# 3169651074/real-time-gpu-ray-tracer

Measured on AMD Instinct MI355X. Metric: Mrays/sec + ms/frame, 1920×1080 1spp primary+shadow, 1/2/4/8 MI355X, higher is better.
Workload: dtype f32; 1 GPU; C2: demo + 68x1024 tris (69,632; bunny stand-in), 1080p 1spp primary+shadow; width=1920, height=1080, spp=1, depth=2, triangles=69633, instances=73, blas_node_pairs=69159, parallelism=single-gpu, overlap_lanes=4, lane_streams=the scene's own (overlap -1: lanes and staging picked by the library), hw_queues=4, tile=32, threshold=auto (64 at depth x spp <= 2, else 40), kernel=FAST persistent, bvh=sah, frames=animated (Main.cu updateInstance), per-frame TLAS rebuild + upload, pipelined

## Files before the change

### real-time-gpu-ray-tracer_amd/csrc/layout.hpp

```cpp
#pragma once
#include <stdint.h>

#include "../../include/rt.h"

namespace rtamd {

constexpr uint32_t REF_LEAF = 1u << 31;
constexpr uint32_t REF_BLAS = 1u << 30;
constexpr uint32_t REF_INDEX_MASK = (1u << 30) - 1u;
constexpr uint32_t REF_START_MASK = (1u << 26) - 1u;
constexpr uint32_t REF_EMPTY = 0xFFFFFFFFu;
constexpr uint32_t MAX_LEAF_SLOTS = 1u << 26;

__host__ __device__ inline uint32_t make_interior_ref(uint32_t pair, bool blas) {
    return (blas ? REF_BLAS : 0u) | (pair & REF_INDEX_MASK);
}
__host__ __device__ inline uint32_t make_leaf_ref(uint32_t start, uint32_t count, uint32_t ptype, bool blas) {
    return REF_LEAF | (blas ? REF_BLAS : 0u) | ((ptype & 3u) << 28) | (((count - 1u) & 3u) << 26) |
           (start & REF_START_MASK);
}
__host__ __device__ inline uint32_t ref_leaf_start(uint32_t r) { return r & REF_START_MASK; }
__host__ __device__ inline uint32_t ref_leaf_count(uint32_t r) { return ((r >> 26) & 3u) + 1u; }
__host__ __device__ inline uint32_t ref_leaf_type(uint32_t r) { return (r >> 28) & 3u; }

// ... 146 lines not shown

constexpr uint32_t FASTDIV_BITS = 27;
struct FastDiv {
    uint32_t d, m, s;
    __host__ __device__ uint32_t div(uint32_t n) const { return (uint32_t)(((uint64_t)n * m) >> s); }
};
inline FastDiv make_fastdiv(uint32_t d) {
    uint32_t l = 0;
    while (l < 31 && (1u << l) < d) l++;
    const uint32_t s = FASTDIV_BITS + l;
    return FastDiv{d, (uint32_t)(((1ull << s) + d - 1) / d), s};
}

struct OutputGPU {
    uint8_t *rgba;
    float *rgb;
    uint32_t units;
    uint32_t units_x;
    uint32_t tile_w, tile_h, tile_rank, tile_count, tiles_x;
    FastDiv div_units_x, div_upt, div_upr, div_tiles_x;
    uint32_t queue_parts;
    uint32_t grab;
    uint32_t supertile;
    unsigned long long *timeline;
    uint32_t *costmap;
    const uint32_t *order;
    uint32_t *unit_cost;
    uint32_t leaf_early;
};
struct RayQueryGPU {
    const float *rays;
    const float *tmax;
    uint32_t n;
    rt_hit *hits;
    float *t;
    uint8_t *occluded;
    uint32_t *head;
};
constexpr uint32_t QUERY_PARTS = 8;
constexpr uint32_t QUEUE_STRIDE = 32;
constexpr uint32_t QUEUE_MAX_PARTS = 8;
constexpr uint32_t QUEUE_WORDS = 2 * QUEUE_MAX_PARTS * QUEUE_STRIDE;
constexpr uint32_t SCHED_CLASSES = 16;

__host__ __device__ inline uint32_t cost_class(uint32_t c) {
    const uint64_t x = (uint64_t)c + 64u;
    const int k = (63 - __builtin_clzll(x * x)) - 12;
    return (SCHED_CLASSES - 1) - (uint32_t)(k < 0 ? 0 : (k > (int)SCHED_CLASSES - 1 ? (int)SCHED_CLASSES - 1 : k));
}
__host__ __device__ inline uint32_t split_log2(uint32_t cls, uint32_t k_half, uint32_t k_quarter) {
    const uint32_t k = (SCHED_CLASSES - 1) - cls;
    return k >= k_quarter ? 2u : (k >= k_half ? 1u : 0u);
}
constexpr uint32_t TIMELINE_WORDS = 20;

enum CounterSlot : uint32_t {
    CNT_RAYS = 0, CNT_PIXELS, CNT_PAIRS, CNT_TRI, CNT_SPHQUAD, CNT_QUAD, CNT_INST, CNT_HITS, CNT_OVERFLOW, CNT_NUM
};

}
```

### real-time-gpu-ray-tracer_amd/csrc/shade.hpp

```cpp

struct Surface { f3 p, n; uint32_t material; uint32_t orig; uint32_t member; };

template <bool LDSS = false, int RAW = 2>
__device__ __forceinline__ Surface finalize(const SceneGPU &sc, const f3 &wo, const f3 &wd, const Hit &h) {
#if !RT_EXACT
    const InstCold IC = LDSS ? lds_or_global(sc.lds_icold, sc.inst_cold, h.inst) : sc.inst_cold[h.inst];
#else
    const InstCold &IC = sc.inst_cold[h.inst];
#endif
    f3 lo, ld;
#if !RT_EXACT
    if (LDSS) {
        const InstRec I = load_inst<true>(sc, h.inst);
        const float inv[12] = {I.i0.x, I.i0.y, I.i0.z, I.i0.w, I.i1.x, I.i1.y, I.i1.z, I.i1.w,
                               I.i2.x, I.i2.y, I.i2.z, I.i2.w};
        lo = xf_point(inv, wo); ld = xf_vector(inv, wd);
    } else
#endif
    {
        const InstHot &I = sc.inst_hot[h.inst];
        lo = xf_point(I.inv, wo); ld = xf_vector(I.inv, wd);
    }
    const f3 p = add(lo, scl(ld, h.t));
    f3 n;
    Surface s;
    if (h.ptype == RT_PRIM_TRIANGLE) {
        f3 n0, n1, n2;
        if (RAW == 1 || (RAW == 2 && sc.raw_tris)) {
            const TriHot &H = sc.tri_hot[h.slot];
            s.orig = __float_as_uint(H.pad0);
            s.member = __float_as_uint(H.pad1);
            const rt_triangle &R = sc.raw_tris[s.orig];
            if (R.has_normals) {
                n0 = mk(R.normal[0].x, R.normal[0].y, R.normal[0].z);
                n1 = mk(R.normal[1].x, R.normal[1].y, R.normal[1].z);
                n2 = mk(R.normal[2].x, R.normal[2].y, R.normal[2].z);
            } else {
                n0 = tri_face_normal(ld3(H.e1), ld3(H.e2)); n1 = n0; n2 = n0;
            }
            s.material = R.material_type == RT_MAT_ROUGH ? R.material_index
                                                         : ((sc.rough_count + R.material_index) | MAT_METAL_BIT);
        } else {
            const TriCold &T = sc.tri_cold[h.slot];
            n0 = ld3(T.n0); n1 = ld3(T.n1); n2 = ld3(T.n2);
            s.material = T.material; s.orig = T.orig_index; s.member = T.pad;
        }
        const f3 nn = unit(add(add(scl(n0, (1.0f - h.u) - h.v), scl(n1, h.u)), scl(n2, h.v)));
        n = dot(ld, nn) < 0.0f ? nn : neg(nn);
    } else if (h.ptype == RT_PRIM_SPHERE) {
#if !RT_EXACT
        const SphereHot S = LDSS ? lds_or_global(sc.lds_sph_hot, sc.sph_hot, h.slot) : sc.sph_hot[h.slot];
        const PrimCold C = LDSS ? lds_or_global(sc.lds_sph_cold, sc.sph_cold, h.slot) : sc.sph_cold[h.slot];
#else
        const SphereHot &S = sc.sph_hot[h.slot];
        const PrimCold &C = sc.sph_cold[h.slot];
#endif
        const f3 outward = unit(sub(p, ld3(S.center)));
        n = dot(ld, outward) < 0.0f ? outward : neg(outward);
        s.material = C.material; s.orig = C.orig_index; s.member = 0u;
    } else {
#if !RT_EXACT
        const float4 qn4 = LDSS && sc.lds_q_hot != LDS_NONE ? lds_scene[sc.lds_q_hot + h.slot * LDS_QPRIM_F4]
                                                              : reinterpret_cast<const float4 *>(sc.quad_hot + h.slot)[0];
        const PrimCold C = LDSS ? lds_or_global(sc.lds_q_cold, sc.quad_cold, h.slot) : sc.quad_cold[h.slot];
        const f3 qn = mk(qn4.x, qn4.y, qn4.z);
#else
        const QuadHot &Q = sc.quad_hot[h.slot];
        const PrimCold &C = sc.quad_cold[h.slot];
        const f3 qn = ld3(Q.n);
#endif
        n = dot(ld, qn) < 0.0f ? qn : neg(qn);
        s.material = C.material; s.orig = C.orig_index; s.member = 0u;
    }
    s.p = xf_point(IC.fwd, p);
    s.n = unit(xf_vector(IC.nrm, n));
    return s;
}

template <bool COUNT>
__device__ f3 ray_color(const SceneGPU &sc, const CameraGPU &cam, f3 o, f3 d, Rng &rng, Trav &T, SEnt *spill,
                        LaneCount &cnt, uint32_t &rays) {
    f3 result = mk(1.0f, 1.0f, 1.0f);
    for (uint32_t depth = 0; depth < cam.depth; depth++) {
        Hit h;
        rays++;
        if (trace<COUNT, XD_ALL>(sc, o, d, h, T, spill, cnt)) {
            if (COUNT) cnt.hits++;
            const Surface s = finalize(sc, o, d, h);
            const float4 m = reinterpret_cast<const float4 *>(sc.materials)[s.material & ~MAT_METAL_BIT];
            const f3 albedo = mk(m.x, m.y, m.z);
            f3 out;
            if (!(s.material & MAT_METAL_BIT)) {
                out = add(s.n, random_space_vector(rng));
                if (f_eq(dot(out, out), FZERO * FZERO)) out = s.n;
            } else {
                out = unit(sub(d, scl(s.n, 2.0f * dot(d, s.n))));
                if (m.w > 0.0f) out = add(out, scl(random_space_vector(rng), m.w));
                if (!(dot(out, s.n) > 0.0f)) return result;
            }
            o = s.p; d = out;
            result = mul(result, albedo);
        } else {
            result = mul(result, ld3(cam.background));
            break;
        }
    }
    return result;
}

__device__ __forceinline__ uint32_t wave_sum(uint32_t v) {
#pragma unroll
    for (int off = 32; off > 0; off >>= 1) v += __shfl_xor(v, off, 64);
    return v;
}

template <bool COUNT>
__device__ __forceinline__ void flush_counts(unsigned long long *counters, const LaneCount &cnt, int lane) {
    if (COUNT) {
        const uint32_t a = wave_sum(cnt.pairs), b = wave_sum(cnt.tri), c = wave_sum(cnt.sq), d = wave_sum(cnt.inst),
                       e = wave_sum(cnt.overflow), f = wave_sum(cnt.quad), g = wave_sum(cnt.hits);
        if (lane == 0) {
            atomicAdd(&counters[CNT_PAIRS], (unsigned long long)a);
            atomicAdd(&counters[CNT_TRI], (unsigned long long)b);
            atomicAdd(&counters[CNT_SPHQUAD], (unsigned long long)c);
            atomicAdd(&counters[CNT_INST], (unsigned long long)d);
            atomicAdd(&counters[CNT_OVERFLOW], (unsigned long long)e);
            atomicAdd(&counters[CNT_QUAD], (unsigned long long)f);
            atomicAdd(&counters[CNT_HITS], (unsigned long long)g);
        }
// ... 76 lines not shown
```

### real-time-gpu-ray-tracer_amd/csrc/trace_kernel.hip

```cpp
#include <hip/hip_runtime.h>
#include <stdint.h>

#include <atomic>

#include "launch.hpp"
#include "layout.hpp"
#include "../../include/rt.h"

#ifndef RT_EXACT
#error "compile with -DRT_EXACT=0 or 1"
#endif

#ifndef RT_FAST_IEEE
#define RT_FAST_IEEE 1
#endif
#if RT_EXACT
#define RT_SUFFIX(n) n##_exact
#elif RT_FAST_IEEE
#define RT_SUFFIX(n) n##_fast
#else
#define RT_SUFFIX(n) n##_fastmath
#endif

namespace rtamd {
// ... 200 lines not shown
                    const uint32_t m = k - sc * st * h;
                    const uint32_t u = (r0 + sr * st + m / w) * W + sc * st + m % w;
                    pool_next = u * 64u;
                    pool_end = pool_next + 64u;
                }
            }
            const uint32_t take = min(n_need, pool_end - pool_next);
            const uint32_t rank = __popcll(need & ((1ull << lane) - 1ull));
            DIAG_T(t_lanes);
            if (!has && rank < take) {
                uint32_t px, py, oi;
                item = pool_next + rank;
                if (map_item(out, cam, item, px, py, oi)) {
                    has = true;
                    const uint32_t pixel = cam.pitch * py + px;
                    rng.init((uint64_t)pixel ^ cam.frame_seed, pixel);
                    acc = mk(0.0f, 0.0f, 0.0f);
                    thr = mk(1.0f, 1.0f, 1.0f);
                    sample = 0; depth = 0;
                    px_steps = 0;
                    f3 o, d;
                    camera_ray(cam, px, py, 0, rng, o, d);
                    trav_init<XBOX(WIDE)>(T, root, o, d);
                    pixels++;
                }
            }
            DIAG_ADD(pc.claim, t_lanes);
            pool_next += take;
            need = __ballot(!has);
        }
        DIAG_ADD(pc.refill, t_refill);
        if (!__any(has)) {
            if (exhausted) break;
            continue;
        }
        for (;;) {
            const uint64_t tr = __ballot(T.tracing);
            if (tr == 0) break;
            const uint64_t want = __ballot(!T.tracing && (has || !exhausted));
            if ((uint32_t)__popcll(want) >= threshold) break;
            spec_round<COUNT, WIDE>(T, sc, spill, cnt, pc, px_steps, COUNT || track, out.leaf_early);
            n_rounds++;
        }
        n_shades++;
        DIAG_T(t_shade);
        bool fin = false;
        if (RT_DIAG) pc.lanes_shade += (unsigned long long)__popcll(__ballot(has && !T.tracing));
        if (has && !T.tracing) {
            rays++;
            bool path_done;
            f3 no = T.wr.o, nd = T.wr.d;
            if (T.found) {
                if (COUNT) cnt.hits++;
                const Surface s = finalize<WIDE != 0, RAW>(sc, T.wr.o, T.wr.d, T.hit);
                DIAG_WAIT_VM();
                DIAG_T(t_hit);
                const uint32_t mi = s.material & ~MAT_METAL_BIT;
                const float4 m = mat_lds ? lds_mat[mi] : reinterpret_cast<const float4 *>(sc.materials)[mi];
                bool absorbed = false;
                if (!(s.material & MAT_METAL_BIT)) {
                    if (depth + 1 < cam.depth || sample + 1 < S2) {
                        nd = add(s.n, random_space_vector(rng));
                        if (f_eq(dot(nd, nd), FZERO * FZERO)) nd = s.n;
                    }
                } else {
                    nd = unit(sub(T.wr.d, scl(s.n, 2.0f * dot(T.wr.d, s.n))));
                    if (m.w > 0.0f) nd = add(nd, scl(random_space_vector(rng), m.w));
                    absorbed = !(dot(nd, s.n) > 0.0f);
                }
                DIAG_ADD(pc.hit, t_hit);
                if (absorbed) {
                    path_done = true;
                } else {
                    thr = mul(thr, mk(m.x, m.y, m.z));
                    no = s.p;
                    depth++;
                    path_done = depth >= cam.depth;
                }
            } else {
                thr = mul(thr, ld3(cam.background));
                path_done = true;
            }
            if (path_done) {
                acc = add(acc, thr);
                sample++;
                uint32_t px, py, oi;
                map_item(out, cam, item, px, py, oi);
                if (sample < S2) {
                    thr = mk(1.0f, 1.0f, 1.0f);
                    depth = 0;
                    camera_ray(cam, px, py, sample, rng, no, nd);
                } else {
                    write_pixel(out, oi, scl(acc, cam.recip_sqrt * cam.recip_sqrt));
                    if (COUNT && out.costmap) out.costmap[oi] = px_steps;
                    has = false;
                    fin = true;
                }
            }
            if (has) trav_init<XBOX(WIDE)>(T, root, no, nd);
        }
        if (track && fin) {
            const uint32_t u = item >> 6;
            if (u != pend_unit) {
                if (pend_cost) unit_cost_flush(out.unit_cost, pend_unit, pend_cost);
                pend_unit = u;
                pend_cost = 0;
            }
            pend_cost = pend_cost + px_steps + 1u;
        }
        DIAG_ADD(pc.shade, t_shade);
    }

    if (track && pend_cost) unit_cost_flush(out.unit_cost, pend_unit, pend_cost);
    const uint32_t wr = wave_sum(rays);
    const uint32_t wp = wave_sum(pixels);
    flush_counts<COUNT>(counters, cnt, lane);
    if (lane == 0) {
        atomicAdd(&counters[CNT_RAYS], (unsigned long long)wr);
        atomicAdd(&counters[CNT_PIXELS], (unsigned long long)wp);
        if (out.timeline) {
            const uint32_t wv = (uint32_t)((const unsigned long long *)T.stk.lds - &lds_stack[0][0]) >> 6;
            unsigned long long *w = out.timeline + (unsigned long long)TIMELINE_WORDS * (blockIdx.x * (BLOCK / 64) + wv);
            w[0] = t_start;
            w[1] = __builtin_amdgcn_s_memrealtime();
            w[2] = ((unsigned long long)hw_id() << 32) | xcc;
            w[3] = wp;
            w[4] = t_exhaust;
            w[5] = n_rounds;
            w[6] = n_shades;
            w[7] = n_grabs;
            w[8] = pc.refill;
            w[9] = pc.interior;
            w[10] = pc.leaf;
            w[11] = pc.shade;
            w[12] = pc.iters;
            w[13] = pc.refill_iters;
            w[14] = pc.claim;
            w[15] = pc.hit;
            w[16] = pc.lanes_interior;
            w[17] = pc.lanes_leaf_tlas;
            w[18] = pc.lanes_leaf_blas;
            w[19] = pc.lanes_shade;
        }
    }
}

template <bool COUNT, int WPE, int WIDE = 0, int RAW = 2>
__global__ __launch_bounds__(BLOCK) __attribute__((amdgpu_waves_per_eu(WPE > 0 ? WPE : 1)))
void render_persistent_kernel(SceneGPU sc, CameraGPU cam, OutputGPU out, uint32_t *queue, uint32_t threshold,
                              unsigned long long *counters) {
    render_persistent_body<COUNT, WIDE, RAW>(sc, cam, out, queue, threshold, counters);
}

__global__ __launch_bounds__(BLOCK) void trace_rays_kernel(SceneGPU sc, const float *rays, uint32_t n, rt_hit *hits) {
    __shared__ unsigned long long lds_stack[LDS_DEPTH][BLOCK];
    const uint32_t i = blockIdx.x * BLOCK + threadIdx.x;
    if (i >= n) return;
    Trav T;
    T.stk.lds = (LdsU2 *)&lds_stack[0][threadIdx.x];
    alignas(16) SEnt spill[SPILL_DEPTH];
    LaneCount cnt = {};
    const f3 o = mk(rays[6 * i], rays[6 * i + 1], rays[6 * i + 2]);
    const f3 d = mk(rays[6 * i + 3], rays[6 * i + 4], rays[6 * i + 5]);
    Hit h;
    rt_hit r;
    if (trace<false, XD_ALL>(sc, o, d, h, T, spill, cnt)) {
        const Surface s = finalize(sc, o, d, h);
        r.t = h.t; r.instance = s.member ? s.member - 1u : (sc.inst_by_slot ? sc.tlas_slots[h.inst] : h.inst);
        r.primitive_type = h.ptype; r.primitive_index = s.orig;
        r.point.x = s.p.x; r.point.y = s.p.y; r.point.z = s.p.z;
        r.normal.x = s.n.x; r.normal.y = s.n.y; r.normal.z = s.n.z;
        const bool metal = (s.material & MAT_METAL_BIT) != 0;
        r.material_type = metal ? RT_MAT_METAL : RT_MAT_ROUGH;
        r.material_index = (s.material & ~MAT_METAL_BIT) - (metal ? sc.rough_count : 0u);
    } else {
        r.t = __builtin_huge_valf(); r.instance = 0xFFFFFFFFu; r.primitive_type = 0; r.primitive_index = 0;
        r.point.x = r.point.y = r.point.z = 0.0f; r.normal.x = r.normal.y = r.normal.z = 0.0f;
        r.material_type = 0; r.material_index = 0;
    }
    hits[i] = r;
}


__global__ __launch_bounds__(BLOCK) void box_test_kernel(const float *boxes, const float *rays, const float *tmaxs, uint32_t n,
                                                         uint32_t mode, uint8_t *hit, float *te) {
    const uint32_t i = blockIdx.x * BLOCK + threadIdx.x;
    if (i >= n) return;
    float b[6];
    for (int c = 0; c < 6; c++) b[c] = boxes[6 * (size_t)i + c];
    RayP r;
    r.o = mk(rays[6 * (size_t)i], rays[6 * (size_t)i + 1], rays[6 * (size_t)i + 2]);
    r.d = mk(rays[6 * (size_t)i + 3], rays[6 * (size_t)i + 4], rays[6 * (size_t)i + 5]);
    const float tmax = tmaxs[i];
    float e = 0.0f;
    bool h = false;
#if RT_EXACT
// ... 128 lines not shown
```

### real-time-gpu-ray-tracer_amd/csrc/traverse.hpp

```cpp

struct Hit {
    float t;
    uint32_t inst;
    uint32_t ptype;
    uint32_t slot;
    float u, v;
};

struct Trav {
    RayP wr, lr;
    float tmax;
    uint32_t cur;
    float curT;
    uint32_t pleaf;
    uint32_t cur_inst;
    Hit hit;
    bool found;
    bool tracing;
    Stack stk;
};

__device__ __forceinline__ bool pop_keep(const Trav &T, float tn, uint32_t ref) {
#if !RT_EXACT
    return cons_lo(tn, (ref & REF_BLAS) ? T.lr.pad : T.wr.pad) < T.tmax;
// ... 69 lines not shown
        float e0 = 0.0f, e1 = 0.0f;
        bool h0, h1;
        const uint4 D = pair_test<COUNT, XB>(T, sc, cur, cnt, h0, h1, e0, e1);
        if (h0 && h1) {
            const bool right_near = e0 > e1;
            stack_push(T.stk, spill, right_near ? D.x : D.y, right_near ? e0 : e1, cnt);
            T.cur = right_near ? D.y : D.x;
            return;
        }
        if (h0) { T.cur = D.x; return; }
        if (h1) { T.cur = D.y; return; }
    } else if (!(cur & REF_BLAS)) {
        const uint32_t start = ref_leaf_start(cur), count = ref_leaf_count(cur);
        if (count > 1) stack_push(T.stk, spill, make_leaf_ref(start + 1, count - 1, 0, false), -__builtin_huge_valf(), cnt);
        T.cur_inst = sc.inst_by_slot ? start : sc.tlas_slots[start];
        const InstHot &I = sc.inst_hot[T.cur_inst];
        if (COUNT) cnt.inst++;
        float te;
        if (enter_instance<XB>(T, I.inv, I.root_box, te)) { T.cur = I.root_ref; return; }
    } else {
        const uint32_t start = ref_leaf_start(cur), count = ref_leaf_count(cur), type = ref_leaf_type(cur);
        for (uint32_t k = 0; k < count; k++) {
            const uint32_t slot = start + k;
            float t = 0.0f, u = 0.0f, v = 0.0f;
            bool h;
            if (type == RT_PRIM_TRIANGLE) {
                if (COUNT) cnt.tri++;
                h = tri_test(sc.tri_hot[slot], T.lr, TMIN, T.tmax, t, u, v);
            } else if (type == RT_PRIM_SPHERE) {
                if (COUNT) cnt.sq++;
                h = sphere_test(sc.sph_hot[slot], T.lr, TMIN, T.tmax, t);
            } else {
                if (COUNT) { cnt.sq++; cnt.quad++; }
                h = quad_test(sc.quad_hot[slot], T.lr, TMIN, T.tmax, t, u, v);
            }
            if (h) accept(T, t, type, slot, u, v);
        }
    }
    while (!T.stk.empty()) {
        const SEnt e = stack_pop(T.stk, spill);
        if (pop_keep(T, __uint_as_float(e.tn), e.ref)) { T.cur = e.ref; return; }
    }
    T.tracing = false;
}

__device__ __forceinline__ void pop_next(Trav &T, const SEnt *spill) {
    while (!T.stk.empty()) {
        const SEnt e = stack_pop(T.stk, spill);
        const float tn = __uint_as_float(e.tn);
        if (pop_keep(T, tn, e.ref)) { T.cur = e.ref; T.curT = tn; return; }
    }
    T.cur = REF_NONE;
}

#if !RT_EXACT
__shared__ float4 lds_scene[LDS_SCENE_F4];

struct InstRec { float4 i0, i1, i2, box01, box2ref; };
template <bool LDSS>
__device__ __forceinline__ InstRec load_inst(const SceneGPU &sc, uint32_t i) {
    InstRec r;
    if (LDSS && sc.lds_insts) {
        const float4 *p = lds_scene + sc.lds_quads * LDS_QUAD_F4 + i * LDS_INST_F4;
        r.i0 = p[0]; r.i1 = p[1]; r.i2 = p[2]; r.box01 = p[3]; r.box2ref = p[4];
    } else {
        const float4 *p = reinterpret_cast<const float4 *>(sc.inst_hot + i);
        r.i0 = p[0]; r.i1 = p[1]; r.i2 = p[2]; r.box01 = p[3]; r.box2ref = p[4];
    }
    return r;
}
__device__ __forceinline__ void lds_scene_fill(const SceneGPU &sc) {
    const uint32_t nq = sc.lds_quads * LDS_QUAD_F4, ni = sc.lds_insts * LDS_INST_F4;
    const float4 *q = reinterpret_cast<const float4 *>(sc.tlas_quads);
    for (uint32_t i = threadIdx.x; i < nq; i += BLOCK) {
        const uint32_t k = i / LDS_QUAD_F4, j = i - k * LDS_QUAD_F4;
        lds_scene[i] = q[k * 8 + j];
    }
    const float4 *h = reinterpret_cast<const float4 *>(sc.inst_hot);
    for (uint32_t i = threadIdx.x; i < ni; i += BLOCK) lds_scene[nq + i] = h[i];
    const auto copy = [](uint32_t at, const void *src, uint32_t n4) {
        if (at == LDS_NONE) return;
        const float4 *p = reinterpret_cast<const float4 *>(src);
        for (uint32_t i = threadIdx.x; i < n4; i += BLOCK) lds_scene[at + i] = p[i];
    };
    copy(sc.lds_icold, sc.inst_cold, sc.instance_count * LDS_ICOLD_F4);
    copy(sc.lds_sph_hot, sc.sph_hot, sc.lds_sph_cold - sc.lds_sph_hot);
    copy(sc.lds_sph_cold, sc.sph_cold, sc.lds_sph_cold - sc.lds_sph_hot);
    copy(sc.lds_q_hot, sc.quad_hot, (sc.lds_q_cold - sc.lds_q_hot));
    copy(sc.lds_q_cold, sc.quad_cold, (sc.lds_q_cold - sc.lds_q_hot) / LDS_QPRIM_F4);
    const float4 *bq = reinterpret_cast<const float4 *>(sc.blas_quads + sc.lds_bq0);
    for (uint32_t i = threadIdx.x; i < sc.lds_bqn * LDS_QUAD_F4; i += BLOCK) {
        const uint32_t k = i / LDS_QUAD_F4, j = i - k * LDS_QUAD_F4;
        lds_scene[sc.lds_bq_at + i] = bq[k * 8 + j];
    }
}
template <typename R>
__device__ __forceinline__ R lds_or_global(uint32_t at, const R *g, uint32_t k) {
    constexpr uint32_t N4 = sizeof(R) / 16;
    R r;
    float4 *d = reinterpret_cast<float4 *>(&r);
    if (at != LDS_NONE) {
#pragma unroll
        for (uint32_t j = 0; j < N4; j++) d[j] = lds_scene[at + k * N4 + j];
    } else {
        const float4 *p = reinterpret_cast<const float4 *>(g + k);
#pragma unroll
// ... 36 lines not shown
    if (!PAIR) {
        float t0 = h[0] ? t[0] : inf, t1 = h[1] ? t[1] : inf, t2 = h[2] ? t[2] : inf, t3 = h[3] ? t[3] : inf;
        uint32_t r0 = R.x, r1 = R.y, r2 = R.z, r3 = R.w;
        const uint32_t nh = (uint32_t)h[0] + (uint32_t)h[1] + (uint32_t)h[2] + (uint32_t)h[3];
        if (nh == 0) { pop_next(T, spill); return; }
        cswap(t0, r0, t1, r1); cswap(t2, r2, t3, r3); cswap(t0, r0, t2, r2); cswap(t1, r1, t3, r3); cswap(t1, r1, t2, r2);
        if (nh > 1) {
            if (T.stk.sp > LDS_DEPTH - 3) stack_page_out(T.stk, spill, cnt);
            SEnt a, b, c;
            a.ref = nh == 4 ? r3 : (nh == 3 ? r2 : r1);
            a.tn = __float_as_uint(nh == 4 ? t3 : (nh == 3 ? t2 : t1));
            b.ref = nh == 4 ? r2 : r1;
            b.tn = __float_as_uint(nh == 4 ? t2 : t1);
            c.ref = r1;
            c.tn = __float_as_uint(t1);
            stack_push3(T.stk, a, b, c, nh - 1u);
        }
        T.cur = r0;
        T.curT = t0;
        return;
    }
    const uint32_t na = (uint32_t)h[0] + (uint32_t)h[1], nb = (uint32_t)h[2] + (uint32_t)h[3];
    if (na + nb == 0) { pop_next(T, spill); return; }
    const float u0 = h[0] ? t[0] : inf, u1 = h[1] ? t[1] : inf, u2 = h[2] ? t[2] : inf, u3 = h[3] ? t[3] : inf;
    const bool sa = u0 > u1, sb = u2 > u3;
    const float a0t = sa ? u1 : u0, a1t = sa ? u0 : u1, b0t = sb ? u3 : u2, b1t = sb ? u2 : u3;
    const uint32_t a0r = sa ? R.y : R.x, a1r = sa ? R.x : R.y, b0r = sb ? R.w : R.z, b1r = sb ? R.z : R.w;
    const bool sr = na == 0 || (nb != 0 && pa > pb);
    const float n0t = sr ? b0t : a0t, n1t = sr ? b1t : a1t, f0t = sr ? a0t : b0t, f1t = sr ? a1t : b1t;
    const uint32_t n0r = sr ? b0r : a0r, n1r = sr ? b1r : a1r, f0r = sr ? a0r : b0r, f1r = sr ? a1r : b1r;
    const uint32_t nn = sr ? nb : na, nf = sr ? na : nb;
    const uint32_t npush = nn - 1u + nf;
    if (npush > 0) {
        if (T.stk.sp > LDS_DEPTH - 3) stack_page_out(T.stk, spill, cnt);
        SEnt a, b, c;
        a.ref = nf == 2 ? f1r : (nf == 1 ? f0r : n1r);
        a.tn = __float_as_uint(nf == 2 ? f1t : (nf == 1 ? f0t : n1t));
        b.ref = nf == 2 ? f0r : n1r;
        b.tn = __float_as_uint(nf == 2 ? f0t : n1t);
        c.ref = n1r;
        c.tn = __float_as_uint(n1t);
        stack_push3(T.stk, a, b, c, npush);
    }
    T.cur = n0r;
    T.curT = n0t;
}
#endif

template <bool COUNT, int WIDE = 0>
__device__ __forceinline__ void spec_interior_step(Trav &T, const SceneGPU &sc, SEnt *spill, LaneCount &cnt) {
    const uint32_t cur = T.cur;
#if !RT_EXACT
    if (WIDE) {
        if (!(cur & REF_LEAF)) wide_interior_step<COUNT, (WIDE >= 2), XBOX(WIDE)>(T, sc, spill, cnt);
        else { T.pleaf = cur; pop_next(T, spill); }
        return;
    }
#endif
    if (!(cur & REF_LEAF)) {
        float e0 = 0.0f, e1 = 0.0f;
        bool h0, h1;
        const uint4 D = pair_test<COUNT, XBOX(WIDE)>(T, sc, cur, cnt, h0, h1, e0, e1);
        if (h0 && h1) {
            const bool right_near = e0 > e1;
            stack_push(T.stk, spill, right_near ? D.x : D.y, right_near ? e0 : e1, cnt);
            T.cur = right_near ? D.y : D.x;
            T.curT = right_near ? e1 : e0;
            return;
        }
        if (h0 || h1) {
            T.cur = h0 ? D.x : D.y;
            T.curT = h0 ? e0 : e1;
            return;
        }
        pop_next(T, spill);
    } else {
        T.pleaf = cur;
        pop_next(T, spill);
    }
}

#if RT_EXACT
#define WIDE_LDS_REC(at, arr, k) (arr)[k]
#else
#define WIDE_LDS_REC(at, arr, k) (WIDE ? lds_or_global((at), (arr), (k)) : (arr)[k])
#endif
template <bool COUNT, int WIDE = 0>
__device__ __forceinline__ uint32_t spec_leaf_phase(Trav &T, const SceneGPU &sc, SEnt *spill, LaneCount &cnt) {
    uint32_t leaf = T.pleaf;
    bool chained = false;
    T.pleaf = REF_NONE;
    if (!(leaf & REF_BLAS)) {
        const uint32_t start = ref_leaf_start(leaf), count = ref_leaf_count(leaf);
        if (T.cur != REF_NONE) stack_push(T.stk, spill, T.cur, T.curT, cnt);
        if (count > 1) stack_push(T.stk, spill, make_leaf_ref(start + 1, count - 1, 0, false), -__builtin_huge_valf(), cnt);
        T.cur_inst = sc.inst_by_slot ? start : sc.tlas_slots[start];
        if (COUNT) cnt.inst++;
        float te = 0.0f;
#if !RT_EXACT
        if (WIDE) {
            const InstRec I = load_inst<true>(sc, T.cur_inst);
            asm volatile("" ::"v"(I.i2.x), "v"(I.i2.y), "v"(I.i2.z), "v"(I.i2.w), "v"(I.box2ref.w));
            const float inv[12] = {I.i0.x, I.i0.y, I.i0.z, I.i0.w, I.i1.x, I.i1.y, I.i1.z, I.i1.w,
                                   I.i2.x, I.i2.y, I.i2.z, I.i2.w};
            const float box[6] = {I.box01.x, I.box01.y, I.box01.z, I.box01.w, I.box2ref.x, I.box2ref.y};
            if (enter_instance<XBOX(WIDE)>(T, inv, box, te)) {
                T.cur = __float_as_uint(I.box2ref.w);
                T.curT = te;
                if (RT_CHAIN_ROOT_LEAF && (T.cur & REF_LEAF)) { leaf = T.cur; chained = true; }
            } else {
                pop_next(T, spill);
            }
        } else
#endif
        {
            const InstHot &I = sc.inst_hot[T.cur_inst];
            if (enter_instance<XBOX(WIDE)>(T, I.inv, I.root_box, te)) { T.cur = WIDE ? I.root_ref_wide : I.root_ref; T.curT = te; }
            else pop_next(T, spill);
        }
    }
    if (leaf & REF_BLAS) {
        const uint32_t start = ref_leaf_start(leaf), count = ref_leaf_count(leaf), type = ref_leaf_type(leaf);
        if (type == RT_PRIM_TRIANGLE) {
            for (uint32_t k0 = 0; k0 < count; k0 += TRI_AHEAD) {
                TriHot H[TRI_AHEAD];
#pragma unroll
                for (uint32_t k = 0; k < TRI_AHEAD; k++) {
                    const float *src = sc.tri_hot[start + min(k0 + k, count - 1u)].v0;
                    const float3 a = *reinterpret_cast<const float3 *>(src);
                    const float3 b = *reinterpret_cast<const float3 *>(src + 4);
                    const float3 c = *reinterpret_cast<const float3 *>(src + 8);
                    H[k].v0[0] = a.x; H[k].v0[1] = a.y; H[k].v0[2] = a.z;
                    H[k].e1[0] = b.x; H[k].e1[1] = b.y; H[k].e1[2] = b.z;
                    H[k].e2[0] = c.x; H[k].e2[1] = c.y; H[k].e2[2] = c.z;
                }
#pragma unroll
                for (uint32_t k = 0; k < TRI_AHEAD; k++) {
                    if (k0 + k >= count) break;
                    float t = 0.0f, u = 0.0f, v = 0.0f;
                    if (COUNT) cnt.tri++;
                    if (tri_test(H[k], T.lr, TMIN, T.tmax, t, u, v)) accept(T, t, type, start + k0 + k, u, v);
                }
            }
        } else {
            for (uint32_t k = 0; k < count; k++) {
                const uint32_t slot = start + k;
                float t = 0.0f, u = 0.0f, v = 0.0f;
                bool h;
                if (type == RT_PRIM_SPHERE) {
                    if (COUNT) cnt.sq++;
                    h = sphere_test(WIDE_LDS_REC(sc.lds_sph_hot, sc.sph_hot, slot), T.lr, TMIN, T.tmax, t);
                } else {
                    if (COUNT) { cnt.sq++; cnt.quad++; }
                    h = quad_test(WIDE_LDS_REC(sc.lds_q_hot, sc.quad_hot, slot), T.lr, TMIN, T.tmax, t, u, v);
                }
                if (h) accept(T, t, type, slot, u, v);
            }
        }
        if (chained) pop_next(T, spill);
        else if (T.cur != REF_NONE && !pop_keep(T, T.curT, T.cur)) pop_next(T, spill);
    }
    if (T.cur == REF_NONE) T.tracing = false;
    return chained ? 1u : 0u;
}

#ifndef RT_DIAG
#define RT_DIAG 0
#endif
struct PhaseCycles {
    unsigned long long refill, interior, leaf, shade, iters, refill_iters, claim, hit;
    unsigned long long lanes_interior, lanes_leaf_tlas, lanes_leaf_blas, lanes_shade;
};
__device__ __forceinline__ unsigned long long stamp() {
    unsigned long long t;
    asm volatile("s_memtime %0\n\ts_waitcnt lgkmcnt(0)" : "=s"(t)::"memory");
    return t;
}
#if RT_DIAG
#define DIAG_WAIT_VM() asm volatile("s_waitcnt vmcnt(0)" ::: "memory")
#define DIAG_T(var) const unsigned long long var = stamp()
#define DIAG_ADD(acc, t0) (acc) += stamp() - (t0)
#else
#define DIAG_WAIT_VM() (void)0
#define DIAG_T(var) (void)0
#define DIAG_ADD(acc, t0) (void)0
#endif

template <bool COUNT, int WIDE = 0>
__device__ __forceinline__ void spec_round(Trav &T, const SceneGPU &sc, SEnt *spill, LaneCount &cnt,
                                           PhaseCycles &pc, uint32_t &steps, bool track, uint32_t leaf_early) {
    DIAG_T(t0);
    for (;;) {
        if (T.tracing && T.pleaf == REF_NONE && T.cur == REF_NONE) T.tracing = false;
        const uint64_t looking = __ballot(T.tracing && T.pleaf == REF_NONE);
        if (!looking) break;
        if (leaf_early && (uint32_t)__popcll(looking) <= leaf_early && __any(T.tracing && T.pleaf != REF_NONE)) break;
        const bool active = T.tracing && T.cur != REF_NONE && (!(T.cur & REF_LEAF) || T.pleaf == REF_NONE);
        if (RT_DIAG) pc.lanes_interior += (unsigned long long)__popcll(__ballot(active));
        if (active) {
            spec_interior_step<COUNT, WIDE>(T, sc, spill, cnt);
            if (track) steps++;
        }
        if (RT_DIAG) pc.iters++;
    }
    DIAG_ADD(pc.interior, t0);
    if (RT_DIAG) {
        pc.lanes_leaf_tlas += (unsigned long long)__popcll(__ballot(T.tracing && T.pleaf != REF_NONE && !(T.pleaf & REF_BLAS)));
        pc.lanes_leaf_blas += (unsigned long long)__popcll(__ballot(T.tracing && T.pleaf != REF_NONE && (T.pleaf & REF_BLAS)));
    }
    DIAG_T(t1);
    if (T.tracing && T.pleaf != REF_NONE) {
        const uint32_t chained = spec_leaf_phase<COUNT, WIDE>(T, sc, spill, cnt);
        if (track) steps += 1u + chained;
    }
    DIAG_ADD(pc.leaf, t1);
}

template <bool COUNT, int XB = XD_CULL>
__device__ __forceinline__ bool trace(const SceneGPU &sc, const f3 &o, const f3 &d, Hit &hit, Trav &T, SEnt *spill,
                                      LaneCount &cnt) {
    trav_init<XB>(T, *sc.tlas_root, o, d);
    while (T.tracing) trav_step<COUNT, XB>(T, sc, spill, cnt);
    hit = T.hit;
    return T.found;
}
```

### real-time-gpu-ray-tracer_amd/rtamd/renderer.py

```python
from __future__ import annotations

import ctypes as C
from contextlib import nullcontext as _null_context

import numpy as np

from . import abi

HIT_DTYPE = np.dtype([("t", np.float32), ("instance", np.uint32), ("ptype", np.uint32),
                      ("pindex", np.uint32), ("point", np.float32, 3), ("normal", np.float32, 3),
                      ("mtype", np.uint32), ("midx", np.uint32)])


def hits_to_numpy(hits) -> np.ndarray:
    raw = hits.detach().cpu().numpy() if hasattr(hits, "detach") else np.asarray(hits, np.uint8)
    return np.ascontiguousarray(raw).reshape(-1, HIT_DTYPE.itemsize).view(HIT_DTYPE).reshape(-1).copy()


class Renderer:
    def __init__(self, scene, device: int = 0, update=None):
        self.lib = abi.load_library()
        self.scene = scene
        self._cb = None
        if update is None:
# ... 44 lines not shown
        from .scenes import instance_desc_array
        arr = instance_desc_array(instances)
        abi.check(self.lib, self.lib.rt_scene_update_instances(self.h, first, len(instances), arr))
        return self

    def update(self, frame: int):
        abi.check(self.lib, self.lib.rt_scene_update(self.h, frame))

    def render(self, frame: int = 0, frame_seed: int = 0x5EED, exact: bool = False, count_work: bool = False,
               want_rgb: bool = False, want_rgba: bool = True, skip_update: bool = False,
               tiles=None, rgba8_device=None, rgb32_device=None, stream=None, sync: bool = True,
               keep_counters: bool = False):
        o = abi.RenderOpts()
        o.frame_seed = frame_seed
        o.flags = (abi.RT_RENDER_EXACT if exact else 0) | (abi.RT_RENDER_COUNT_WORK if count_work else 0) | \
                  (abi.RT_RENDER_SKIP_UPDATE if skip_update else 0) | (0 if sync else abi.RT_RENDER_NO_SYNC) | \
                  (abi.RT_RENDER_KEEP_COUNTERS if keep_counters else 0)
        comm = getattr(self, "comm", None)
        if comm is not None and comm[0] != 0:
            want_rgba = False
        if tiles is not None:
            o.tile_w, o.tile_h, o.tile_rank, o.tile_count = tiles
            npix = self.tiles_for_rank(*tiles) * tiles[0] * tiles[1]
            shape = (npix,)
        else:
            shape = (self.height, self.width)
        o.rgba8_device = rgba8_device
        o.rgb32_device = rgb32_device
        o.stream = stream
        rgba = np.zeros(shape + (4,), np.uint8) if (want_rgba and sync) else None
        rgb = np.zeros(shape + (3,), np.float32) if (want_rgb and sync) else None
        st = abi.Stats()
        abi.check(self.lib, self.lib.rt_render(self.h, frame, C.byref(o),
                                               rgba.ctypes.data if rgba is not None else None,
                                               rgb.ctypes.data if rgb is not None else None, C.byref(st)))
        stats = {k: getattr(st, k) for k, _ in abi.Stats._fields_}
        return rgba, rgb, stats

    def collect(self, capacity: int = 256):
        st = abi.Stats()
        ms = (C.c_float * capacity)()
        n = C.c_uint32()
        abi.check(self.lib, self.lib.rt_scene_collect(self.h, C.byref(st), ms, capacity, C.byref(n)))
        return {k: getattr(st, k) for k, _ in abi.Stats._fields_}, [ms[i] for i in range(n.value)]

    def debug_read(self, name: str) -> np.ndarray:
        n = C.c_size_t()
        abi.check(self.lib, self.lib.rt_scene_debug_read(self.h, name.encode(), None, 0, C.byref(n)))
        buf = np.zeros(n.value, np.uint8)
        abi.check(self.lib, self.lib.rt_scene_debug_read(self.h, name.encode(), buf.ctypes.data, n.value, C.byref(n)))
        return buf

    def timeline(self):
        w = self.debug_read("timeline").view(np.uint64).reshape(-1, 20)
        out = np.zeros(len(w), dtype=[("start", np.uint64), ("end", np.uint64), ("xcc", np.uint32),
                                      ("hw_id", np.uint32), ("pixels", np.uint32), ("exhaust", np.uint64),
                                      ("rounds", np.uint32), ("shades", np.uint32), ("grabs", np.uint32),
                                      ("cyc_refill", np.uint64), ("cyc_interior", np.uint64), ("cyc_leaf", np.uint64),
                                      ("cyc_shade", np.uint64), ("iters", np.uint64), ("refill_iters", np.uint64),
                                      ("cyc_lanes", np.uint64), ("cyc_scatter", np.uint64),
                                      ("lanes_interior", np.uint64), ("lanes_leaf_tlas", np.uint64),
                                      ("lanes_leaf_blas", np.uint64), ("lanes_shade", np.uint64)])
        out["start"], out["end"], out["exhaust"] = w[:, 0], w[:, 1], w[:, 4]
        out["xcc"], out["hw_id"], out["pixels"] = w[:, 2] & 0xFFFFFFFF, w[:, 2] >> 32, w[:, 3]
        out["rounds"], out["shades"], out["grabs"] = w[:, 5], w[:, 6], w[:, 7]
        out["cyc_refill"], out["cyc_interior"], out["cyc_leaf"], out["cyc_shade"] = w[:, 8], w[:, 9], w[:, 10], w[:, 11]
        out["iters"], out["refill_iters"] = w[:, 12], w[:, 13]
        out["cyc_lanes"], out["cyc_scatter"] = w[:, 14], w[:, 15]
        out["lanes_interior"], out["lanes_leaf_tlas"], out["lanes_leaf_blas"], out["lanes_shade"] = w[:, 16], w[:, 17], w[:, 18], w[:, 19]
        return out

    def costmap(self):
        return self.debug_read("costmap").view(np.uint32)

    def tiles_for_rank(self, tile_w, tile_h, rank, count):
        return int(self.lib.rt_tiles_for_rank(self.h, tile_w, tile_h, rank, count))

    def assemble_tiles(self, gathered_device, slab_tiles, tile_w, tile_h, tile_count, frame_device, stream=None):
        abi.check(self.lib, self.lib.rt_assemble_tiles(self.h, gathered_device, slab_tiles, tile_w, tile_h,
                                                       tile_count, frame_device, stream))

    @staticmethod
    def comm_unique_id() -> bytes:
        lib = abi.load_library()
        cid = abi.CommId()
        abi.check(lib, lib.rt_comm_unique_id(C.byref(cid)))
        return bytes(bytearray(cid))

    def attach_comm(self, comm_id: bytes, rank: int, world: int, tile_w: int = 64, tile_h: int = 64):
        cid = abi.CommId.from_buffer_copy(bytes(comm_id))
        abi.check(self.lib, self.lib.rt_scene_attach_comm(self.h, C.byref(cid), rank, world, tile_w, tile_h))
        self.comm = (rank, world, tile_w, tile_h)
        return self

    def detach_comm(self):
        abi.check(self.lib, self.lib.rt_scene_detach_comm(self.h))
        self.comm = None
        return self

    def trace_rays(self, rays, exact: bool = False):
        rays = np.ascontiguousarray(rays, np.float32).reshape(-1, 6)
        n = rays.shape[0]
        hits = (abi.Hit * max(1, n))()
        abi.check(self.lib, self.lib.rt_trace_rays(self.h, rays.ctypes.data, n,
                                                   abi.RT_RENDER_EXACT if exact else 0, hits))
        out = np.zeros(n, dtype=[("t", np.float32), ("instance", np.uint32), ("ptype", np.uint32),
                                 ("pindex", np.uint32), ("point", np.float32, 3), ("normal", np.float32, 3),
                                 ("mtype", np.uint32), ("midx", np.uint32)])
        out[:] = np.frombuffer(hits, dtype=out.dtype, count=n)
        return out

    def query_rays(self, rays, tmax=None, *, any_hit: bool = False, exact: bool = False, want_hits: bool = True,
                   stream=None, sync: bool = True):
        import torch

        dev = torch.device("cuda", self.device)
        if stream is None:
            stream = torch.cuda.current_stream(dev)
        ctx = torch.cuda.stream(stream) if isinstance(stream, torch.cuda.Stream) else _null_context()
        uploaded = []

        def device_f32(x, shape, name):
# ... 111 lines not shown
```

Measured before the change: 17530 Mrays/s.

## Skip surface finalize on last-bounce rough hits; split leaf postponement from interior step

On the final bounce of a rough (non-metal) surface, the shader now fetches only the material index and albedo and no longer computes the full surface (hit point and normal transform). It still advances the RNG so the random sequence stays the same. The traversal loop now routes leaf refs into a separate postpone_leaf branch instead of handling them inside spec_interior_step, and it postpones a freshly reached leaf right after the leaf phase. New diagnostic counters and timeline words are also added; they run only when RT_DIAG is set.

```diff
diff --git a/real-time-gpu-ray-tracer_amd/csrc/layout.hpp b/real-time-gpu-ray-tracer_amd/csrc/layout.hpp
--- a/real-time-gpu-ray-tracer_amd/csrc/layout.hpp
+++ b/real-time-gpu-ray-tracer_amd/csrc/layout.hpp
@@ -222,7 +222,7 @@
     const uint32_t k = (SCHED_CLASSES - 1) - cls;
     return k >= k_quarter ? 2u : (k >= k_half ? 1u : 0u);
 }
-constexpr uint32_t TIMELINE_WORDS = 20;
+constexpr uint32_t TIMELINE_WORDS = 24;
 
 enum CounterSlot : uint32_t {
     CNT_RAYS = 0, CNT_PIXELS, CNT_PAIRS, CNT_TRI, CNT_SPHQUAD, CNT_QUAD, CNT_INST, CNT_HITS, CNT_OVERFLOW, CNT_NUM
diff --git a/real-time-gpu-ray-tracer_amd/csrc/shade.hpp b/real-time-gpu-ray-tracer_amd/csrc/shade.hpp
--- a/real-time-gpu-ray-tracer_amd/csrc/shade.hpp
+++ b/real-time-gpu-ray-tracer_amd/csrc/shade.hpp
@@ -75,6 +75,24 @@
     s.p = xf_point(IC.fwd, p);
     s.n = unit(xf_vector(IC.nrm, n));
     return s;
+}
+
+template <bool LDSS = false, int RAW = 2>
+__device__ __forceinline__ uint32_t hit_material(const SceneGPU &sc, const Hit &h) {
+    if (h.ptype == RT_PRIM_TRIANGLE) {
+        if (RAW == 1 || (RAW == 2 && sc.raw_tris)) {
+            const rt_triangle &R = sc.raw_tris[__float_as_uint(sc.tri_hot[h.slot].pad0)];
+            return R.material_type == RT_MAT_ROUGH ? R.material_index : ((sc.rough_count + R.material_index) | MAT_METAL_BIT);
+        }
+        return sc.tri_cold[h.slot].material;
+    }
+#if !RT_EXACT
+    if (LDSS) {
+        if (h.ptype == RT_PRIM_SPHERE) return lds_or_global(sc.lds_sph_cold, sc.sph_cold, h.slot).material;
+        return lds_or_global(sc.lds_q_cold, sc.quad_cold, h.slot).material;
+    }
+#endif
+    return (h.ptype == RT_PRIM_SPHERE ? sc.sph_cold : sc.quad_cold)[h.slot].material;
 }
 
 template <bool COUNT>
diff --git a/real-time-gpu-ray-tracer_amd/csrc/trace_kernel.hip b/real-time-gpu-ray-tracer_amd/csrc/trace_kernel.hip
--- a/real-time-gpu-ray-tracer_amd/csrc/trace_kernel.hip
+++ b/real-time-gpu-ray-tracer_amd/csrc/trace_kernel.hip
@@ -276,30 +276,39 @@
             f3 no = T.wr.o, nd = T.wr.d;
             if (T.found) {
                 if (COUNT) cnt.hits++;
-                const Surface s = finalize<WIDE != 0, RAW>(sc, T.wr.o, T.wr.d, T.hit);
-                DIAG_WAIT_VM();
-                DIAG_T(t_hit);
-                const uint32_t mi = s.material & ~MAT_METAL_BIT;
-                const float4 m = mat_lds ? lds_mat[mi] : reinterpret_cast<const float4 *>(sc.materials)[mi];
-                bool absorbed = false;
-                if (!(s.material & MAT_METAL_BIT)) {
-                    if (depth + 1 < cam.depth || sample + 1 < S2) {
+                if (RT_DIAG) pc.hits++;
+                const uint32_t material = hit_material<WIDE != 0, RAW>(sc, T.hit);
+                const uint32_t mi = material & ~MAT_METAL_BIT;
+                if (depth + 1 >= cam.depth && !(material & MAT_METAL_BIT)) {
+                    if (RT_DIAG) pc.hits_last_rough++;
+                    const float4 m = mat_lds ? lds_mat[mi] : reinterpret_cast<const float4 *>(sc.materials)[mi];
+                    if (sample + 1 < S2) (void)random_space_vector(rng);
+                    thr = mul(thr, mk(m.x, m.y, m.z));
+                    depth++;
+                    path_done = true;
+                } else {
+                    const Surface s = finalize<WIDE != 0, RAW>(sc, T.wr.o, T.wr.d, T.hit);
+                    DIAG_WAIT_VM();
+                    DIAG_T(t_hit);
+                    const float4 m = mat_lds ? lds_mat[mi] : reinterpret_cast<const float4 *>(sc.materials)[mi];
+                    bool absorbed = false;
+                    if (!(s.material & MAT_METAL_BIT)) {
                         nd = add(s.n, random_space_vector(rng));
                         if (f_eq(dot(nd, nd), FZERO * FZERO)) nd = s.n;
+                    } else {
+                        nd = unit(sub(T.wr.d, scl(s.n, 2.0f * dot(T.wr.d, s.n))));
+                        if (m.w > 0.0f) nd = add(nd, scl(random_space_vector(rng), m.w));
+                        absorbed = !(dot(nd, s.n) > 0.0f);
                     }
-                } else {
-                    nd = unit(sub(T.wr.d, scl(s.n, 2.0f * dot(T.wr.d, s.n))));
-                    if (m.w > 0.0f) nd = add(nd, scl(random_space_vector(rng), m.w));
-                    absorbed = !(dot(nd, s.n) > 0.0f);
-                }
-                DIAG_ADD(pc.hit, t_hit);
-                if (absorbed) {
-                    path_done = true;
-                } else {
-                    thr = mul(thr, mk(m.x, m.y, m.z));
-                    no = s.p;
-                    depth++;
-                    path_done = depth >= cam.depth;
+                    DIAG_ADD(pc.hit, t_hit);
+                    if (absorbed) {
+                        path_done = true;
+                    } else {
+                        thr = mul(thr, mk(m.x, m.y, m.z));
+                        no = s.p;
+                        depth++;
+                        path_done = depth >= cam.depth;
+                    }
                 }
             } else {
                 thr = mul(thr, ld3(cam.background));
@@ -365,7 +374,15 @@
             w[17] = pc.lanes_leaf_tlas;
             w[18] = pc.lanes_leaf_blas;
             w[19] = pc.lanes_shade;
-        }
+            w[20] = pc.lanes_postpone;
+            w[21] = pc.iters_idle;
+        }
+    }
+    if (RT_DIAG && out.timeline) {
+        const uint32_t wv = (uint32_t)((const unsigned long long *)T.stk.lds - &lds_stack[0][0]) >> 6;
+        unsigned long long *w = out.timeline + (unsigned long long)TIMELINE_WORDS * (blockIdx.x * (BLOCK / 64) + wv);
+        atomicAdd(&w[22], pc.hits);
+        atomicAdd(&w[23], pc.hits_last_rough);
     }
 }
 
diff --git a/real-time-gpu-ray-tracer_amd/csrc/traverse.hpp b/real-time-gpu-ray-tracer_amd/csrc/traverse.hpp
--- a/real-time-gpu-ray-tracer_amd/csrc/traverse.hpp
+++ b/real-time-gpu-ray-tracer_amd/csrc/traverse.hpp
@@ -145,6 +145,10 @@
     }
     T.cur = REF_NONE;
 }
+__device__ __forceinline__ void postpone_leaf(Trav &T, const SEnt *spill) {
+    T.pleaf = T.cur;
+    pop_next(T, spill);
+}
 
 #if !RT_EXACT
 __shared__ float4 lds_scene[LDS_SCENE_F4];
@@ -287,32 +291,26 @@
     const uint32_t cur = T.cur;
 #if !RT_EXACT
     if (WIDE) {
-        if (!(cur & REF_LEAF)) wide_interior_step<COUNT, (WIDE >= 2), XBOX(WIDE)>(T, sc, spill, cnt);
-        else { T.pleaf = cur; pop_next(T, spill); }
+        wide_interior_step<COUNT, (WIDE >= 2), XBOX(WIDE)>(T, sc, spill, cnt);
         return;
     }
 #endif
-    if (!(cur & REF_LEAF)) {
-        float e0 = 0.0f, e1 = 0.0f;
-        bool h0, h1;
-        const uint4 D = pair_test<COUNT, XBOX(WIDE)>(T, sc, cur, cnt, h0, h1, e0, e1);
-        if (h0 && h1) {
-            const bool right_near = e0 > e1;
-            stack_push(T.stk, spill, right_near ? D.x : D.y, right_near ? e0 : e1, cnt);
-            T.cur = right_near ? D.y : D.x;
-            T.curT = right_near ? e1 : e0;
-            return;
-        }
-        if (h0 || h1) {
-            T.cur = h0 ? D.x : D.y;
-            T.curT = h0 ? e0 : e1;
-            return;
-        }
-        pop_next(T, spill);
-    } else {
-        T.pleaf = cur;
-        pop_next(T, spill);
-    }
+    float e0 = 0.0f, e1 = 0.0f;
+    bool h0, h1;
+    const uint4 D = pair_test<COUNT, XBOX(WIDE)>(T, sc, cur, cnt, h0, h1, e0, e1);
+    if (h0 && h1) {
+        const bool right_near = e0 > e1;
+        stack_push(T.stk, spill, right_near ? D.x : D.y, right_near ? e0 : e1, cnt);
+        T.cur = right_near ? D.y : D.x;
+        T.curT = right_near ? e1 : e0;
+        return;
+    }
+    if (h0 || h1) {
+        T.cur = h0 ? D.x : D.y;
+        T.curT = h0 ? e0 : e1;
+        return;
+    }
+    pop_next(T, spill);
 }
 
 #if RT_EXACT
@@ -405,6 +403,7 @@
 struct PhaseCycles {
     unsigned long long refill, interior, leaf, shade, iters, refill_iters, claim, hit;
     unsigned long long lanes_interior, lanes_leaf_tlas, lanes_leaf_blas, lanes_shade;
+    unsigned long long lanes_postpone, iters_idle, hits, hits_last_rough;
 };
 __device__ __forceinline__ unsigned long long stamp() {
     unsigned long long t;
@@ -431,9 +430,19 @@
         if (!looking) break;
         if (leaf_early && (uint32_t)__popcll(looking) <= leaf_early && __any(T.tracing && T.pleaf != REF_NONE)) break;
         const bool active = T.tracing && T.cur != REF_NONE && (!(T.cur & REF_LEAF) || T.pleaf == REF_NONE);
-        if (RT_DIAG) pc.lanes_interior += (unsigned long long)__popcll(__ballot(active));
-        if (active) {
+        const bool node = active && !(T.cur & REF_LEAF);
+        if (RT_DIAG) {
+            pc.lanes_interior += (unsigned long long)__popcll(__ballot(active));
+            if (!__ballot(node)) pc.iters_idle++;
+        }
+        if (node) {
             spec_interior_step<COUNT, WIDE>(T, sc, spill, cnt);
+            if (track) steps++;
+        }
+        const bool leaf = active && T.pleaf == REF_NONE && (T.cur & REF_LEAF) && T.cur != REF_NONE;
+        if (RT_DIAG) pc.lanes_postpone += (unsigned long long)__popcll(__ballot(leaf));
+        if (leaf) {
+            postpone_leaf(T, spill);
             if (track) steps++;
         }
         if (RT_DIAG) pc.iters++;
@@ -447,6 +456,10 @@
     if (T.tracing && T.pleaf != REF_NONE) {
         const uint32_t chained = spec_leaf_phase<COUNT, WIDE>(T, sc, spill, cnt);
         if (track) steps += 1u + chained;
+        if (T.tracing && (T.cur & REF_LEAF) && T.cur != REF_NONE) {
+            postpone_leaf(T, spill);
+            if (track) steps++;
+        }
     }
     DIAG_ADD(pc.leaf, t1);
 }
diff --git a/real-time-gpu-ray-tracer_amd/rtamd/renderer.py b/real-time-gpu-ray-tracer_amd/rtamd/renderer.py
--- a/real-time-gpu-ray-tracer_amd/rtamd/renderer.py
+++ b/real-time-gpu-ray-tracer_amd/rtamd/renderer.py
@@ -120,7 +120,7 @@
         return buf
 
     def timeline(self):
-        w = self.debug_read("timeline").view(np.uint64).reshape(-1, 20)
+        w = self.debug_read("timeline").view(np.uint64).reshape(-1, 24)
         out = np.zeros(len(w), dtype=[("start", np.uint64), ("end", np.uint64), ("xcc", np.uint32),
                                       ("hw_id", np.uint32), ("pixels", np.uint32), ("exhaust", np.uint64),
                                       ("rounds", np.uint32), ("shades", np.uint32), ("grabs", np.uint32),
@@ -128,7 +128,9 @@
                                       ("cyc_shade", np.uint64), ("iters", np.uint64), ("refill_iters", np.uint64),
                                       ("cyc_lanes", np.uint64), ("cyc_scatter", np.uint64),
                                       ("lanes_interior", np.uint64), ("lanes_leaf_tlas", np.uint64),
-                                      ("lanes_leaf_blas", np.uint64), ("lanes_shade", np.uint64)])
+                                      ("lanes_leaf_blas", np.uint64), ("lanes_shade", np.uint64),
+                                      ("lanes_postpone", np.uint64), ("iters_idle", np.uint64),
+                                      ("hits", np.uint64), ("hits_last_rough", np.uint64)])
         out["start"], out["end"], out["exhaust"] = w[:, 0], w[:, 1], w[:, 4]
         out["xcc"], out["hw_id"], out["pixels"] = w[:, 2] & 0xFFFFFFFF, w[:, 2] >> 32, w[:, 3]
         out["rounds"], out["shades"], out["grabs"] = w[:, 5], w[:, 6], w[:, 7]
@@ -136,6 +138,7 @@
         out["iters"], out["refill_iters"] = w[:, 12], w[:, 13]
         out["cyc_lanes"], out["cyc_scatter"] = w[:, 14], w[:, 15]
         out["lanes_interior"], out["lanes_leaf_tlas"], out["lanes_leaf_blas"], out["lanes_shade"] = w[:, 16], w[:, 17], w[:, 18], w[:, 19]
+        out["lanes_postpone"], out["iters_idle"], out["hits"], out["hits_last_rough"] = w[:, 20], w[:, 21], w[:, 22], w[:, 23]
         return out
 
     def costmap(self):
```

New measurement: 18100 Mrays/s (median of 6 runs). 1.03x the previous value.
